# SAIC-MONTREAL/multimodal-dynamics

Measured on AMD Instinct MI355X. Metric: visuotactile samples/sec (train) + ELBO vs CPU ref, cnn-mvae 64x64 bs256 @1/2/4/8 GPU, higher is better.
Workload: dtype f32x3; 1 GPU; cnn-mvae visuotactile+pose 64x64, bs=256 per GPU, fp32 storage and results, GEMMs in the fp32x3 arithmetic (exact three-term bf16 split of the fp32 operands, six of nine products on the bf16 matrix cores, fp32 accumulate; error vs fp64 <= native fp32 MFMA), seq_modeling train step (7 subset ELBOs + backward + Adam), BASELINE configs[1]; global_batch=256, parallelism=dp1, bn=local, launch=hip_graph

## Files before the change

### include/mmdyn_hip.h

```cpp
#ifndef MMDYN_HIP_H
#define MMDYN_HIP_H

#include <stdint.h>

#ifdef __cplusplus
extern "C" {
#endif

#define MMDYN_OK 0
#define MMDYN_ERR_SHAPE (-1)
#define MMDYN_ERR_NULL (-2)
#define MMDYN_ERR_RANGE (-3)

#define MMDYN_ACT_NONE 0
#define MMDYN_ACT_SWISH 1
#define MMDYN_ACT_RELU 2

#define MMDYN_DENSE 0
#define MMDYN_CONV 1
#define MMDYN_TCONV_S2P1 2
#define MMDYN_IM2COL3 3

#define MMDYN_TCONV_S1P0 4

// ... 26 lines not shown
int mmdyn_igemm_stat_tiles(int mode, int G, int Bg, int Hi, int Wi, int Cin, int Ho, int Wo, int N);
int mmdyn_igemm_stat_tiles_bf16(int mode, int G, int Bg, int Hi, int Wi, int Cin, int Ho, int Wo, int N);
int mmdyn_igemm_stat_tiles_mx(int mode, int G, int Bg, int Hi, int Wi, int Cin, int Ho, int Wo, int N, int flags);
int mmdyn_igemm_slab_floats_mx(int mode, int G, int Bg, int Hi, int Wi, int Cin, int Ho, int Wo, int N, int flags);
int mmdyn_igemm_nt_grouped(const void* A, const void* Bp, const float* bias, void* C, void* C_act, const void* u, int G,
                           int rows, int K, int N, int act, int flags, void* stream);
int mmdyn_splitk_reduce(const float* ws, const float* bias, float* C, float* C_act, int splitk,
                        int rows, int N, int act, void* stream);

int mmdyn_wgrad_tn(const float* D, const float* Gt, float* partial, int mode, int Bt, int Hr, int Wr,
                   int Cd, int Hi, int Wi, int Cg, int stride, int offset, int chunks, void* stream);
int mmdyn_wgrad_tn_bf16(const float* D, const float* Gt, float* partial, int mode, int Bt, int Hr, int Wr,
                        int Cd, int Hi, int Wi, int Cg, int stride, int offset, int chunks, void* stream);
int mmdyn_wgrad_tn_f16(const float* D, const float* Gt, float* partial, int mode, int Bt, int Hr, int Wr,
                       int Cd, int Hi, int Wi, int Cg, int stride, int offset, int chunks, void* stream);
int mmdyn_wgrad_tn_grouped(const void* D, const void* Gt, float* partial, int G, int rows, int Cd, int Cg, int chunks,
                           int flags, void* stream);
int mmdyn_wgrad_out3_bn(const void* y, const float* mean, const float* rstd, const float* gamma, const float* beta,
                        const float* Gt, float* partial, int G, int Bg, int Hr, int chunks, int y_b16, void* stream);
int mmdyn_wgrad_chunks(int mode, int rows, int Cd, int Cg);
int mmdyn_wgrad_chunks_mx(int mode, int rows, int Cd, int Cg, int flags);
int mmdyn_wgrad_reduce(const float* partial, float* canon, int chunks, int taps, int Cd, int Cg,
                       int cg_canon, int perm, float beta, void* stream);

int mmdyn_pack_conv_weight(const float* Wc, float* P, int d0, int d1, int swap, void* stream);
int mmdyn_repack2d(const float* in, float* out, int rows_in, int cols_in, int rows_out, int cols_out,
                   int mode, void* stream);

int mmdyn_repack2d_ld(const float* in, float* out, int rows_in, int cols_in, int rows_out, int cols_out,
                      int ld_out, int mode, void* stream);
int mmdyn_pack_conv_weight_b16(const float* Wc, void* P, int d0, int d1, int swap, int half, void* stream);
int mmdyn_repack2d_ld_b16(const float* in, void* out, int rows_in, int cols_in, int rows_out, int cols_out,
                          int ld_out, int mode, int half, void* stream);
typedef struct {
  const float* src;
  float* dst;
  int kind, rows_in, cols_in, rows_out, cols_out, ld_out;
  int dst_bf16;
} mmdyn_pack_entry;
int mmdyn_pack_plan(const mmdyn_pack_entry* plan_dev, int n, void* stream);

int mmdyn_im2col_nchw3(const float* x, float* col, int Bt, int H, int W, void* stream);
int mmdyn_col2im_k4(const float* col, float* out, int Bt, int Hi, int Wi, int Ho, int Wo, int C,
                    int ldcol, int stride, int pad, int tap_major, void* stream);

int mmdyn_tconv_out3_fwd(const float* a, const float* w, float* out, int Bt, int Hi, int Wi, void* stream);
// ... 268 lines not shown
```

### multimodal-dynamics_amd/csrc/wgrad_geom.h

```cpp
#pragma once
#include "common.h"

struct WgradGeom {
  int d_b16, g_b16;
  int f16;
  int mode;
  int rows;
  int Hr, Wr, Cd;
  int Hi, Wi, Cg;
  int rs, ro;
  int ntaps, chunks, rows_per_chunk;
  int groups;
  int x3;
  int pre;
};

#ifdef MMDYN_LAB
int mmdyn_wgrad_ws_try(const float* D, const float* Gt, float* partial, const WgradGeom& g, hipStream_t st);
#else
static inline int mmdyn_wgrad_ws_try(const float*, const float*, float*, const WgradGeom&, hipStream_t) { return 1; }
#endif

int mmdyn_wgrad_p3_try(const void* D, const void* Gt, float* partial, const WgradGeom& g, int Bt, hipStream_t st);
int mmdyn_wgrad_p3_chunks(int rows, int Cd, int Cg);
```

### multimodal-dynamics_amd/csrc/wgrad_tn.hip

```cpp
#include <stdlib.h>
#include "common.h"
#include "wgrad_geom.h"

namespace {


constexpr int RK = 32;

typedef __bf16 bf16x4 __attribute__((ext_vector_type(4)));
typedef short s16x4 __attribute__((ext_vector_type(4)));
typedef _Float16 f16x4 __attribute__((ext_vector_type(4)));
__device__ __forceinline__ f16x4 pack4_f16(float a, float b, float c, float d) {
  f16x4 r;
  r[0] = (_Float16)a; r[1] = (_Float16)b; r[2] = (_Float16)c; r[3] = (_Float16)d;
  return r;
}
__device__ __forceinline__ s16x4 pack4_bf16(float a, float b, float c, float d) {
  bf16x4 r;
  r[0] = (__bf16)a; r[1] = (__bf16)b; r[2] = (__bf16)c; r[3] = (__bf16)d;
  return __builtin_bit_cast(s16x4, r);
}

template <int BX> struct x3_ld { static constexpr int v = (BX == 32) ? 32 : BX + 32; };
template <int MODE, int BD, int BG, int WD, int WG, int WK, bool BF16, int ST, bool X3 = false, int PRE = 0>
__global__ __launch_bounds__(256) void wgrad_tn_kernel(const float* __restrict__ D,
                                                       const float* __restrict__ Gt,
                                                       float* __restrict__ partial, const WgradGeom g) {
  static_assert(!X3 || (!BF16 && ST == 0 && WK == 1 && MODE != MMDYN_IM2COL3), "the three-term split is a variant of the fp32 kernel");
  static_assert(PRE == 0 || X3, "operands that arrive split belong to the three-term split arithmetic");
  constexpr bool PD = (PRE & 1) != 0, PG = (PRE & 2) != 0;
  constexpr int DT = WD / 32, GT = WG / 32;
  constexpr int WAVES_G = BG / WG;
  constexpr int WAVES_DG = (BD / WD) * WAVES_G;
  static_assert(WAVES_DG * WK == 4, "4 waves per block");
  constexpr int KPW = (RK / 2) / WK;
  constexpr int DV = BD / 4, GV = BG / 4;
  constexpr int D_LOADS = (RK * DV) / 256, G_LOADS = (RK * GV) / 256;
  static_assert(D_LOADS >= 1 && G_LOADS >= 1, "tile too small for 256 threads");

  extern __shared__ __attribute__((aligned(16))) char smem[];
  float* Ds = reinterpret_cast<float*>(smem);
  float* Gs = Ds + RK * BD;
  constexpr int LDD = x3_ld<BD>::v, LDG = x3_ld<BG>::v;
  bf16_t* Ds16 = reinterpret_cast<bf16_t*>(smem);
  bf16_t* Gs16 = Ds16 + 3 * RK * LDD;

  const int tid = threadIdx.x, lane = tid & 63, wave = tid >> 6;
  const int wk = wave / WAVES_DG, wdg = wave % WAVES_DG;
  const int wd = wdg / WAVES_G, wg = wdg % WAVES_G;
  const int tiles_g = g.Cg / BG;
  const int td = blockIdx.x / tiles_g, tg = blockIdx.x - td * tiles_g;
  const int cd0 = td * BD, cg0 = tg * BG;
  const int tap = blockIdx.y;
  const int ngrp = g.groups > 1 ? g.groups : 1;
  const int zb = gridDim.z / ngrp;
  const int grp = blockIdx.z / zb, chunk = blockIdx.z - grp * zb;
  const int dh = (MODE == MMDYN_CONV) ? (tap >> 2) : 0;
  const int dw = (MODE == MMDYN_CONV) ? (tap & 3) : 0;
  const int HWr = g.Hr * g.Wr;

  const int row_begin = grp * g.rows + chunk * g.rows_per_chunk;
  const int row_end = min((grp + 1) * g.rows, row_begin + g.rows_per_chunk);

  const float inv_hw = 1.0f / (float)HWr, inv_w = 1.0f / (float)g.Wr;
  auto fdiv = [](int n, int d, float inv, int& q, int& r) {
    q = (int)((float)n * inv);
    r = n - q * d;
    if (r < 0) { q -= 1; r += d; }
    if (r >= d) { q += 1; r -= d; }
  };
  f32x4 rd[D_LOADS], rg[G_LOADS];
  constexpr int DV8 = BD / 8, GV8 = BG / 8;
  constexpr int D_LOADS8 = (RK * DV8) / 256, G_LOADS8 = (RK * GV8) / 256;
  static_assert(PRE == 0 || (D_LOADS8 >= 1 && G_LOADS8 >= 1), "plane granules: tile too small for 256 threads");
  u32x4 pd[PD ? D_LOADS8 : 1][3], pg[PG ? G_LOADS8 : 1][3];
  unsigned okd = 0, okg = 0;
  auto gload = [&](int r0) {
    if constexpr (PD) {
#pragma unroll
      for (int i = 0; i < D_LOADS8; ++i) {
        const int idx = tid + 256 * i;
        const int r = idx / DV8, v = idx - r * DV8;
        const int row = r0 + r;
        const bool ok = row < row_end;
        const bf16_t* b = reinterpret_cast<const bf16_t*>(D) + (size_t)(ok ? row : 0) * 3 * g.Cd + cd0 + v * 8;
// ... 139 lines not shown
    }
#pragma unroll
    for (int i = 0; i < D_LOADS; ++i)
      reinterpret_cast<f32x4*>(Ds)[tid + 256 * i] = ((okd >> i) & 1u) ? rd[i] : zero;
#pragma unroll
    for (int i = 0; i < G_LOADS; ++i) {
      const unsigned m = okg >> (4 * i);
      f32x4 v;
      v[0] = (m & 1u) ? rg[i][0] : 0.f;
      v[1] = (m & 2u) ? rg[i][1] : 0.f;
      v[2] = (m & 4u) ? rg[i][2] : 0.f;
      v[3] = (m & 8u) ? rg[i][3] : 0.f;
      reinterpret_cast<f32x4*>(Gs)[tid + 256 * i] = v;
    }
  };

  f32x16 acc[DT][GT];
#pragma unroll
  for (int a = 0; a < DT; ++a)
#pragma unroll
    for (int b = 0; b < GT; ++b)
#pragma unroll
      for (int e = 0; e < 16; ++e) acc[a][b][e] = 0.f;

  const int h = lane >> 5, cl = lane & 31;
  if (row_begin < row_end) {
    gload(row_begin);
    lds_store();
    __syncthreads();
    for (int r0 = row_begin; r0 < row_end; r0 += RK) {
      gload(r0 + RK);
      __builtin_amdgcn_sched_barrier(0);
      if constexpr (X3) {
        const int gq = lane >> 4, tq = (lane >> 2) & 3, tp = lane & 3;
        const int trow = 8 * (gq >> 1) + tq, tcol = 16 * (gq & 1) + 4 * tp;
        typedef __attribute__((address_space(3))) s16x4* lds_s16x4_p;
        typedef __bf16 xb16x8 __attribute__((ext_vector_type(8)));
        auto frag = [&](const bf16_t* tile, int ld, int col0, int k0) {
          const s16x4 lo = __builtin_amdgcn_ds_read_tr16_b64_v4i16((lds_s16x4_p)(&tile[(k0 + trow) * ld + col0 + tcol]));
          const s16x4 hi = __builtin_amdgcn_ds_read_tr16_b64_v4i16((lds_s16x4_p)(&tile[(k0 + trow + 4) * ld + col0 + tcol]));
          typedef short s16x8 __attribute__((ext_vector_type(8)));
          const s16x8 v = {lo[0], lo[1], lo[2], lo[3], hi[0], hi[1], hi[2], hi[3]};
          return __builtin_bit_cast(xb16x8, v);
        };
#pragma unroll
        for (int kc = 0; kc < 2; ++kc) {
// ... 47 lines not shown
            pb[b] = pack4_bf16(p[0], p[BG], p[2 * BG], p[3 * BG]);
          }
#pragma unroll
          for (int a = 0; a < DT; ++a)
#pragma unroll
            for (int b = 0; b < GT; ++b)
              acc[a][b] = __builtin_amdgcn_mfma_f32_32x32x8bf16_1k(pa[a], pb[b], acc[a][b], 0, 0, 0);
          }
        }
      } else
#pragma unroll
      for (int kk = wk * KPW; kk < (wk + 1) * KPW; ++kk) {
        float af[DT], bf[GT];
#pragma unroll
        for (int a = 0; a < DT; ++a) af[a] = Ds[(2 * kk + h) * BD + wd * WD + a * 32 + cl];
#pragma unroll
        for (int b = 0; b < GT; ++b) bf[b] = Gs[(2 * kk + h) * BG + wg * WG + b * 32 + cl];
#pragma unroll
        for (int a = 0; a < DT; ++a)
#pragma unroll
          for (int b = 0; b < GT; ++b)
            acc[a][b] = __builtin_amdgcn_mfma_f32_32x32x2f32(af[a], bf[b], acc[a][b], 0, 0, 0);
      }
      __builtin_amdgcn_sched_barrier(0);
      __syncthreads();
      lds_store();
      __syncthreads();
    }
  }

  float* out = partial + ((size_t)(((chunk * WK + wk) * ngrp + grp) * g.ntaps + tap) * g.Cd) * g.Cg;
#pragma unroll
  for (int a = 0; a < DT; ++a)
#pragma unroll
    for (int e = 0; e < 16; ++e) {
      const int cd = cd0 + wd * WD + a * 32 + (e & 3) + 8 * (e >> 2) + 4 * h;
#pragma unroll
      for (int b = 0; b < GT; ++b) {
        const int cg = cg0 + wg * WG + b * 32 + cl;
        out[(size_t)cd * g.Cg + cg] = acc[a][b][e];
      }
    }
}

typedef __bf16 wb16x8 __attribute__((ext_vector_type(8)));
typedef _Float16 wf16x8 __attribute__((ext_vector_type(8)));
typedef float wacc16_t __attribute__((ext_vector_type(16)));
template <bool H16> __device__ __forceinline__ wacc16_t mfma16(wb16x8 a, wb16x8 b, wacc16_t c) {
  if constexpr (H16)
    return __builtin_amdgcn_mfma_f32_32x32x16_f16(__builtin_bit_cast(wf16x8, a), __builtin_bit_cast(wf16x8, b), c, 0, 0, 0);
  else
// ... 624 lines not shown
  for (int64_t tile = blockIdx.x; tile < ntiles; tile += gridDim.x) {
    const int64_t i = tile * 32 + il;
    float s0 = 0.f, s1 = 0.f, s2 = 0.f, s3 = 0.f;
    if (i < slab) {
      int c = cl;
      for (; c + 24 < chunks; c += 32) {
        s0 += partial[(size_t)c * slab + i];
        s1 += partial[(size_t)(c + 8) * slab + i];
        s2 += partial[(size_t)(c + 16) * slab + i];
        s3 += partial[(size_t)(c + 24) * slab + i];
      }
      for (; c < chunks; c += 8) s0 += partial[(size_t)c * slab + i];
    }
    red[cl][il] = (s0 + s1) + (s2 + s3);
    __syncthreads();
    if (cl == 0 && i < slab) {
      float s = 0.f;
#pragma unroll
      for (int k = 0; k < 8; ++k) s += red[k][il];
      int cg = (int)(i % Cg);
      int64_t t = i / Cg;
      int cd = (int)(t % Cd);
      int tap = (int)(t / Cd);
      if (cg < cg_canon) {
        int64_t o;
        if (perm == 0) {
          o = ((int64_t)cd * cg_canon + cg) * taps + tap;
        } else if (perm == 1) {
          int hw = cg / 256, ch = cg - hw * 256;
          o = (int64_t)cd * cg_canon + ch * 25 + hw;
        } else {
          int hw = cd / 256, ch = cd - hw * 256;
          o = (int64_t)(ch * 25 + hw) * cg_canon + cg;
        }
        canon[o] = (beta != 0.f) ? (beta * canon[o] + s) : s;
      }
    }
    __syncthreads();
  }
}

__global__ __launch_bounds__(256) void wgrad_reduce_vec_kernel(const float* __restrict__ partial,
                                                               float* __restrict__ canon, int chunks, int taps,
                                                               int Cd, int Cg, int cg_canon, int perm, float beta) {
  const int64_t slab = (int64_t)taps * Cd * Cg, nvec = slab >> 2;
  for (int64_t v = blockIdx.x * (int64_t)blockDim.x + threadIdx.x; v < nvec; v += (int64_t)gridDim.x * blockDim.x) {
    const int64_t i = v << 2;
    f32x4 s = {0.f, 0.f, 0.f, 0.f};
#pragma unroll 8
    for (int c = 0; c < chunks; ++c) s += *reinterpret_cast<const f32x4*>(partial + (size_t)c * slab + i);
    const int cg0 = (int)(i % Cg);
    const int64_t t = i / Cg;
    const int cd = (int)(t % Cd), tap = (int)(t / Cd);
#pragma unroll
    for (int k = 0; k < 4; ++k) {
      const int cg = cg0 + k;
      if (cg >= cg_canon) continue;
      int64_t o;
      if (perm == 0) {
        o = ((int64_t)cd * cg_canon + cg) * taps + tap;
      } else if (perm == 1) {
        int hw = cg / 256, ch = cg - hw * 256;
        o = (int64_t)cd * cg_canon + ch * 25 + hw;
      } else {
        int hw = cd / 256, ch = cd - hw * 256;
        o = (int64_t)(ch * 25 + hw) * cg_canon + cg;
      }
      canon[o] = (beta != 0.f) ? (beta * canon[o] + s[k]) : s[k];
    }
  }
}

template <int BD, int BG, int WD, int WG, int WK>
static int launch_b16(const float* D, const float* Gt, float* partial, WgradGeom g, hipStream_t st) {
  const int zblocks = g.chunks / WK;
  int rpc = ceil_div(g.rows, zblocks);
  g.rows_per_chunk = ceil_div(rpc, RK) * RK;
  dim3 grid((unsigned)((g.Cd / BD) * (g.Cg / BG) * g.ntaps) * (unsigned)((zblocks + 7) / 8 * 8));
#define WGRAD_B16(M, H)                                                                                    \
  hipLaunchKernelGGL((wgrad_b16_kernel<M, BD, BG, WD, WG, WK, H>), grid, dim3(256), 0, st,                 \
                     reinterpret_cast<const bf16_t*>(D), reinterpret_cast<const bf16_t*>(Gt), partial, g)
  if (g.mode == MMDYN_CONV) {
    if (g.f16) WGRAD_B16(MMDYN_CONV, true);
    else WGRAD_B16(MMDYN_CONV, false);
  } else {
    if (g.f16) WGRAD_B16(MMDYN_DENSE, true);
    else WGRAD_B16(MMDYN_DENSE, false);
  }
#undef WGRAD_B16
  MMDYN_LAUNCH_CHECK();
}
// ... 31 lines not shown
      MMDYN_LAUNCH_CHECK();
    }
  }
#define WGRAD_LAUNCH(M, BF, ST_)                                                                                      \
  hipLaunchKernelGGL((wgrad_tn_kernel<M, BD, BG, WD, WG, WK, BF, ST_>), grid, dim3(256), smem, st, D, Gt, partial, g)
#define WGRAD_MODE(M)                                                  \
  do {                                                                 \
    if (bf16 && g.f16 && g.d_b16 && g.g_b16) WGRAD_LAUNCH(M, true, 5); \
    else if (bf16 && g.f16 && g.d_b16) WGRAD_LAUNCH(M, true, 6);       \
    else if (bf16 && g.f16 && g.g_b16) WGRAD_LAUNCH(M, true, 7);       \
    else if (bf16 && g.d_b16 && g.g_b16) WGRAD_LAUNCH(M, true, 1);     \
    else if (bf16 && g.d_b16) WGRAD_LAUNCH(M, true, 2);                \
    else if (bf16 && g.g_b16) WGRAD_LAUNCH(M, true, 3);                \
    else if (bf16 && g.f16) WGRAD_LAUNCH(M, true, 4);                  \
    else if (bf16) WGRAD_LAUNCH(M, true, 0);                           \
    else WGRAD_LAUNCH(M, false, 0);                                    \
  } while (0)
  if (g.mode == MMDYN_CONV) WGRAD_MODE(MMDYN_CONV);
  else if (g.mode == MMDYN_DENSE) WGRAD_MODE(MMDYN_DENSE);
  else if constexpr (BG == 64) WGRAD_MODE(MMDYN_IM2COL3);
  else return MMDYN_ERR_SHAPE;
#undef WGRAD_MODE
#undef WGRAD_LAUNCH
  MMDYN_LAUNCH_CHECK();
}

}

static bool tile_128x64() {
  const char* e = lab_env("MMDYN_WGRAD_128x64");
  return !(e && e[0] == '0');
}

static bool p3_enabled() {
  const char* e = lab_env("MMDYN_WGRAD_P3");
  return !(e && e[0] == '0');
}

static bool p3_asked(bool x3, int pre, int mode) { return x3 && pre == 3 && mode == MMDYN_CONV && p3_enabled(); }

enum WgradFamily {
  WGRAD_TN,
  WGRAD_TN4,
  WGRAD_B16
};
struct WgradRoute {
// ... 157 lines not shown
    if (c > 0) return c;
  }
  return wgrad_chunks_impl(mode, rows, Cd, Cg, (flags & 6) == 6, x3);
}

extern "C" int mmdyn_wgrad_reduce(const float* partial, float* canon, int chunks, int taps, int Cd, int Cg,
                                  int cg_canon, int perm, float beta, void* stream) {
  if (!partial || !canon) return MMDYN_ERR_NULL;
  if (cg_canon > Cg || cg_canon <= 0) return MMDYN_ERR_SHAPE;
  if (perm == 1 && (Cg % 256 || Cg / 256 != 25)) return MMDYN_ERR_SHAPE;
  if (perm == 2 && (Cd % 256 || Cd / 256 != 25)) return MMDYN_ERR_SHAPE;
  int64_t slab = (int64_t)taps * Cd * Cg;
  if (chunks <= 64 && slab >= 65536) {
    hipLaunchKernelGGL(wgrad_reduce_vec_kernel, dim3(ew_grid(slab >> 2)), dim3(256), 0, (hipStream_t)stream, partial,
                       canon, chunks, taps, Cd, Cg, cg_canon, perm, beta);
    MMDYN_LAUNCH_CHECK();
  }
  int64_t ntiles = (slab + 31) / 32;
  int grid = (int)(ntiles < 8192 ? ntiles : 8192);
  hipLaunchKernelGGL(wgrad_reduce_kernel, dim3(grid), dim3(256), 0, (hipStream_t)stream, partial, canon, chunks,
                     taps, Cd, Cg, cg_canon, perm, beta);
  MMDYN_LAUNCH_CHECK();
}
```

### multimodal-dynamics_amd/mmdyn_hip/_lib.py

```python
import ctypes
import os

_HERE = os.path.dirname(os.path.abspath(__file__))
LIB_PATH = os.environ.get("MMDYN_HIP_LIB") or os.path.join(_HERE, "libmmdyn_hip.so")

_P, _I, _L, _F, _Q = ctypes.c_void_p, ctypes.c_int, ctypes.c_int64, ctypes.c_float, ctypes.c_uint64


class PassExperts(ctypes.Structure):
    _fields_ = [("mu", _P * 4), ("lv", _P * 4), ("dmu", _P * 4), ("dlv", _P * 4), ("ld", _I * 4), ("dz", _P * 3),
                ("zdst", _P * 3), ("zpl", _P * 3)]


class PackEntry(ctypes.Structure):
    _fields_ = [("src", _P), ("dst", _P), ("kind", _I), ("rows_in", _I), ("cols_in", _I), ("rows_out", _I),
                ("cols_out", _I), ("ld_out", _I), ("dst_bf16", _I)]


class FeedGroups(ctypes.Structure):
    _fields_ = [("recon", _P * 4), ("obs", _P * 4), ("out", _P * 4), ("row_len", _I * 4), ("logits", _I * 4), ("column", _I * 4)]


class GatherGroups(ctypes.Structure):
    _fields_ = [("src", _P * 4), ("out", _P * 4), ("row_len", _I * 4), ("logits", _I * 4)]
# ... 10 lines not shown
ABI_VERSION = 6

_SIGNATURES = {
    "mmdyn_abi_version": "",
    "mmdyn_igemm_nt": "ppppppp" + "iiiiiiiiiiiiii" + "p",
    "mmdyn_igemm_nt_dgrad_bn": "ppppppppp" + "iiiiiiiiiiii" + "ppp",
    "mmdyn_igemm_nt_dgrad_act": "pppp" + "i" + "iiiiiiiiiii" + "i" + "ppp",
    "mmdyn_igemm_slab_floats": "iiiiiiiii",
    "mmdyn_igemm_nt_bf16": "ppppppp" + "iiiiiiiiiiiiii" + "p",
    "mmdyn_igemm_nt_f16": "ppppppp" + "iiiiiiiiiiiiii" + "p",
    "mmdyn_igemm_stat_tiles": "iiiiiiiii",
    "mmdyn_igemm_stat_tiles_bf16": "iiiiiiiii",
    "mmdyn_igemm_stat_tiles_mx": "iiiiiiiiii",
    "mmdyn_igemm_slab_floats_mx": "iiiiiiiiii",
    "mmdyn_igemm_nt_grouped": "pppppp" + "iiiiii" + "p",
    "mmdyn_splitk_reduce": "pppp" + "iiii" + "p",
    "mmdyn_wgrad_tn": "ppp" + "iiiiiiiiiii" + "p",
    "mmdyn_wgrad_tn_bf16": "ppp" + "iiiiiiiiiii" + "p",
    "mmdyn_wgrad_tn_f16": "ppp" + "iiiiiiiiiii" + "p",
    "mmdyn_wgrad_tn_grouped": "ppp" + "iiiiii" + "p",
    "mmdyn_wgrad_chunks": "iiii",
    "mmdyn_wgrad_chunks_mx": "iiiii",
    "mmdyn_wgrad_reduce": "pp" + "iiiiii" + "f" + "p",
    "mmdyn_pack_conv_weight": "pp" + "iii" + "p",
    "mmdyn_repack2d": "pp" + "iiiii" + "p",
    "mmdyn_repack2d_ld": "pp" + "iiiiii" + "p",
    "mmdyn_pack_conv_weight_b16": "pp" + "iiii" + "p",
    "mmdyn_repack2d_ld_b16": "pp" + "iiiiiii" + "p",
    "mmdyn_pack_plan": "p" + "i" + "p",
    "mmdyn_im2col_nchw3": "pp" + "iii" + "p",
    "mmdyn_col2im_k4": "pp" + "iiiiiiiiii" + "p",
    "mmdyn_tconv_out3_fwd": "ppp" + "iii" + "p",
    "mmdyn_tconv_out3_bn_fwd": "ppppppp" + "iiiii" + "p",
    "mmdyn_tconv_out3_bn_bce": "ppppppp" + "i" + "pp" + "i" + "pppp" + "f" + "iiiii" + "p",
    "mmdyn_wgrad_out3_bn": "ppppppp" + "iiiii" + "p",
    "mmdyn_colstats": "pp" + "iii" + "p",
    "mmdyn_colstats_tiles": "i",
    "mmdyn_bn_finalize": "ppppppp" + "iiii" + "ff" + "i" + "pp",
    "mmdyn_bn_swish_fwd": "pppppp" + "iii" + "p",
    "mmdyn_bn_swish_bwd_reduce": "ppppppp" + "iii" + "p",
    "mmdyn_bn_bwd_finalize": "ppppp" + "iii" + "f" + "pp",
    "mmdyn_bn_eval_stats": "pppp" + "ii" + "f" + "p",
    "mmdyn_bn_reduce_partials": "ppp" + "iii" + "p",
    "mmdyn_bn_finalize_sums": "pppppp" + "iii" + "ff" + "i" + "p",
    "mmdyn_bn_bwd_finalize_sums": "pppp" + "ii" + "ff" + "p",
    "mmdyn_bn_swish_bwd_apply": "pppppppp" + "iiii" + "p",
# ... 125 lines not shown
```

### multimodal-dynamics_amd/mmdyn_hip/layers.py

```python
import weakref

import torch

from . import ops
from .ops import ACT_NONE, ACT_SWISH, ACT_RELU, DENSE, CONV, TCONV_S2P1, IM2COL3, TCONV_S1P0
from .models.shapes import BN_EPS, BN_MOMENTUM, FEAT


def _new(like, *shape, dtype=torch.float32):
    if isinstance(like, ops.Planes):
        like = like.t
    return torch.empty(shape, device=like.device, dtype=dtype)


ACT_DTYPE = torch.float32
W_DTYPE = torch.float32


def _act(like, *shape):
    return torch.empty(shape, device=like.device, dtype=ACT_DTYPE)


def _cdiv(a, b):
    return (a + b - 1) // b
# ... 33 lines not shown
    else:
        ops.B.igemm_nt(A, Bp, bias, C, Ca, None, None, DENSE, 1, rows, 1, 1, K, 1, 1, N, N, 1, 0, act, 1)
    return C, Ca


PLANES = True
PLANE_TWIN = {}


def _plane_twin(Wp):
    ent = PLANE_TWIN.get(Wp.data_ptr())
    if ent is None:
        return None
    if ent[0]() is not Wp:
        if ent[0]() is None:
            del PLANE_TWIN[Wp.data_ptr()]
        return None
    return ent[1]


PATCH_PLANES = True
CONV1_PLANES = True
OUT3_RECOMPUTE = True


def _conv3_plane_op(name, switch, S, *tensors):
    if not switch or S != 64 or ACT_DTYPE != torch.float32 or any(t.dtype != torch.float32 for t in tensors):
        return None
    return getattr(ops.B, name, None)


def planes_served(mode, G, Bg, Hi, Cin, Ho, N):
    served = getattr(ops.B, "igemm_planes_served", None) if PLANES else None
    if N == 32 and not PATCH_PLANES:
        return False
    return bool(served is not None and ACT_DTYPE == torch.float32 and served(mode, G, Bg, Hi, Hi, Cin, Ho, Ho, N))


def split_operands(x, Wp, mode, G, Bg, Hi, Cin, Ho, N):
    if isinstance(Wp, ops.Planes):
        return x, Wp
    xin = x.t if isinstance(x, ops.Planes) else x
    if xin.dtype not in (torch.float32, torch.bfloat16) or Wp.dtype != torch.float32 or not planes_served(mode, G, Bg, Hi, Cin, Ho, N):
        if isinstance(x, ops.Planes):
            raise ValueError("mmdyn_hip: a plane operand for a launch the plane-ring kernel does not serve")
        return x, Wp
# ... 221 lines not shown
            _bn_eval_param_grads(y, partial, T, dgamma, dbeta, G, N)
        dy, dyp = _apply_out(y, planes_out)
        ops.backend_op("bn_eval_swish_bwd")(du, None, mean, rstd, bn.gamma, bn.beta, dy, None, G, rows_per_group, N, True, planes=dyp)
        return dy if dyp is None else dyp
    sums = _bn_backward_sums(y, partial, T, dgamma, dbeta, G, N)
    dy, dyp = _apply_out(y, planes_out)
    if dyp is not None:
        ops.B.bn_swish_bwd_apply(du, y, mean, rstd, bn.gamma, bn.beta, sums, None, G, rows_per_group, N, True, planes=dyp)
        return dyp
    ops.B.bn_swish_bwd_apply(du, y, mean, rstd, bn.gamma, bn.beta, sums, dy, G, rows_per_group, N, True)
    return dy


def wgrad(D, Gt, canon, mode, Bt, Hr, Cd, Hi, Cg, stride=1, offset=0, cg_canon=None, perm=0, defer=None):
    if defer is not None:
        defer.append((D, Gt, canon, mode, Bt, Hr, Cd, Hi, Cg, stride, offset, cg_canon, perm))
        return
    rows = Bt * Hr * Hr
    taps = 16 if mode == CONV else 1
    if isinstance(D, ops.Planes) or isinstance(Gt, ops.Planes):
        chunks = ops.B.wgrad_chunks(mode, rows, Cd, Cg, planes=(isinstance(D, ops.Planes), isinstance(Gt, ops.Planes)))
    else:
        chunks = ops.B.wgrad_chunks(mode, rows, Cd, Cg)
    partial = _new(D, chunks, taps, Cd, Cg)
    ops.B.wgrad_tn(D, Gt, partial, mode, Bt, Hr, Hr, Cd, Hi, Hi, Cg, stride, offset, chunks)
    ops.B.wgrad_reduce(partial, canon, chunks, taps, Cd, Cg, Cg if cg_canon is None else cg_canon, perm, 0.0)


def run_deferred_wgrads(queue):
    while queue:
        item = queue.pop(0)
        if item and callable(item[0]):
            item[0](*item[1:])
        else:
            wgrad(*item)


def bn_stats_only(y, partial, T, bn, G, rows_per_group, C, repeat=1):
    if partial is None:
        return _eval_stats(y, bn, G, C)
    return _bn_forward_stats(y, partial, T, bn, G, rows_per_group, C, repeat)


def fuses_last_bn(S):
    return S in (64, 128, 256)

# ... 686 lines not shown
```

### multimodal-dynamics_amd/mmdyn_hip/ops.py

```python
import ctypes

import os

import torch

from . import _lib
from ._lib import PassExperts, FeedGroups, GatherGroups, EnsembleGroups, MAX_PASSES, MAX_EXPERTS, FEED_GROUPS, check

ACT_NONE, ACT_SWISH, ACT_RELU = 0, 1, 2
DENSE, CONV, TCONV_S2P1, IM2COL3, TCONV_S1P0 = 0, 1, 2, 3, 4
ROW_GROUPS_MAX = 8
PLAN_TOP_MAX = 8
REFIT_N_MAX = 4096


def _ptr(t, dtype=torch.float32):
    if t is None:
        return None
    if not t.is_cuda:
        raise RuntimeError("mmdyn_hip: the HIP path needs GPU tensors (got a CPU tensor); there is no CPU fallback")
    if t.dtype != dtype:
        raise TypeError(f"mmdyn_hip: expected {dtype}, got {t.dtype}")
    if not t.is_contiguous():
        raise ValueError("mmdyn_hip: tensor must be contiguous")
# ... 330 lines not shown
                else:
                    ptrs.append(_ptr(t))
            check(self.lib.mmdyn_wgrad_tn_mx(ptrs[0], ptrs[1], _ptr(partial), mode, Bt, Hr, Wr, Cd, Hi, Wi, Cg, stride, offset, chunks,
                                             flags, _stream()), "mmdyn_wgrad_tn_mx")
            return
        (pd, d16), (pg, g16) = _aptr(D), _aptr(Gt)
        if d16 or g16:
            check(self.lib.mmdyn_wgrad_tn_mx(pd, pg, _ptr(partial), mode, Bt, Hr, Wr, Cd, Hi, Wi, Cg, stride, offset, chunks,
                                             self._mx(d16, g16) | (2 if d16 else 0) | (4 if g16 else 0), _stream()),
                  "mmdyn_wgrad_tn_mx")
            return
        if self._x3():
            check(self.lib.mmdyn_wgrad_tn_mx(pd, pg, _ptr(partial), mode, Bt, Hr, Wr, Cd, Hi, Wi, Cg, stride, offset, chunks, 128,
                                             _stream()), "mmdyn_wgrad_tn_mx")
            return
        fn = {"fp32": self.lib.mmdyn_wgrad_tn, "fp16": self.lib.mmdyn_wgrad_tn_f16,
              "fp16s": self.lib.mmdyn_wgrad_tn_f16}.get(self.precision, self.lib.mmdyn_wgrad_tn_bf16)
        check(fn(pd, pg, _ptr(partial), mode, Bt, Hr, Wr, Cd, Hi, Wi, Cg, stride, offset, chunks,
                 _stream()), "mmdyn_wgrad_tn")

    def wgrad_reduce(self, partial, canon, chunks, taps, Cd, Cg, cg_canon, perm, beta):
        check(self.lib.mmdyn_wgrad_reduce(_ptr(partial), _ptr(canon), chunks, taps, Cd, Cg, cg_canon, perm,
                                          float(beta), _stream()), "mmdyn_wgrad_reduce")

    def pack_conv_weight(self, Wc, P, d0, d1, swap):
        pp, p16 = _aptr(P)
        if p16:
            check(self.lib.mmdyn_pack_conv_weight_b16(_ptr(Wc), pp, d0, d1, int(swap), _half(p16), _stream()),
                  "mmdyn_pack_conv_weight_b16")
            return
        check(self.lib.mmdyn_pack_conv_weight(_ptr(Wc), pp, d0, d1, int(swap), _stream()), "mmdyn_pack_conv_weight")

    def repack2d(self, src, dst, rows_in, cols_in, rows_out, cols_out, mode):
        if _is16(dst):
            return self.repack2d_ld(src, dst, rows_in, cols_in, rows_out, cols_out, cols_out, mode)
        check(self.lib.mmdyn_repack2d(_ptr(src), _ptr(dst), rows_in, cols_in, rows_out, cols_out, mode, _stream()),
              "mmdyn_repack2d")

    def repack2d_ld(self, src, dst, rows_in, cols_in, rows_out, cols_out, ld_out, mode):
        _, d16 = _aptr(dst)
        if d16:
            check(self.lib.mmdyn_repack2d_ld_b16(_ptr(src), dst.data_ptr(), rows_in, cols_in, rows_out, cols_out, ld_out, mode,
                                                 _half(d16), _stream()), "mmdyn_repack2d_ld_b16")
            return
        check(self.lib.mmdyn_repack2d_ld(_ptr(src), dst.data_ptr(), rows_in, cols_in, rows_out, cols_out, ld_out, mode,
                                         _stream()), "mmdyn_repack2d_ld")
# ... 966 lines not shown
```

### multimodal-dynamics_amd/mmdyn_hip/profiling.py

```python
import collections

import torch

from . import ops

PAD_CYCLES = 100000
HOST_ONLY = {"igemm_stat_tiles", "colstats_tiles", "wgrad_chunks", "igemm_planes_served"}


def _canon(name, a):
    if name == "igemm_nt_dgrad_bn":
        A, Bp, C, stats, y, mean, rstd, gamma, beta, mode, G, Bg, Hi, Wi, Cin, Ho, Wo, N, stride, offset = a
        name, a = "igemm_nt", (A, Bp, y, C, None, stats, None, mode, G, Bg, Hi, Wi, Cin, Ho, Wo, N, N, stride, offset, 0, 1)
    if name == "igemm_nt_dgrad_act":
        A, Bp, C, u, act, mode, G, Bg, Hi, Wi, Cin, Ho, Wo, N, stride, offset = a
        name, a = "igemm_nt", (A, Bp, u, C, None, None, None, mode, G, Bg, Hi, Wi, Cin, Ho, Wo, N, N, stride, offset, 0, 1)
    if name == "igemm_nt_grouped":
        A, Bp, bias, C, C_act, u, G, rows, K, N, act = a
        name, a = "igemm_nt", (A, Bp, bias if u is None else u, C, C_act, None, None, ops.DENSE, G, rows, 1, 1, K, 1, 1, N, N, 1, 0, act, 1)
    if name == "wgrad_tn_grouped":
        D, Gt, partial, G, rows, Cd, Cg, chunks = a
        name, a = "wgrad_tn", (D, Gt, partial, ops.DENSE, G * rows, 1, 1, Cd, 1, 1, Cg, 1, 0, chunks)
    if name == "wgrad_out3_bn":
        y, mean, rstd, gamma, beta, Gt, partial, G, Bg, Hr, chunks = a
        return "conv3_wgrad", (y, Gt, partial, ops.IM2COL3, G * Bg, Hr, Hr, 32, 2 * Hr, 2 * Hr, 64, 1, 0, chunks)
    if name == "tconv_out3_bn_fwd":
        return "tconv_out3_fwd", a
    if name == "conv3_fwd_planes":
        x, Wp, C, planes, G, Bg, H, act = a
        return "conv3_nt", (x, Wp, None, C, planes, None, None, ops.IM2COL3, G, Bg, H, H, 64, H // 2, H // 2, 32, 32, 1, 0, act, 1)
    if name == "conv3_dgrad_bn_stats":
        x, Wp, stats, y, mean, rstd, gamma, beta, G, Bg, H = a
        return "conv3_nt", (x, Wp, y, None, None, stats, None, ops.IM2COL3, G, Bg, H, H, 64, H // 2, H // 2, 32, 32, 1, 0, 0, 1)
    if name == "conv3_dgrad_bn_apply_planes":
        x, Wp, y, mean, rstd, gamma, beta, sums, planes, G, Bg, H = a
        return "conv3_nt", (x, Wp, y, planes, None, None, None, ops.IM2COL3, G, Bg, H, H, 64, H // 2, H // 2, 32, 32, 1, 0, 0, 1)
    if name == "igemm_nt" and a[7] == ops.IM2COL3 and a[10] in (64, 128, 256) and \
            tuple(a[10:17]) == (a[10], a[10], 64, a[10] // 2, a[10] // 2, 32, 32):
        return "conv3_nt", a
    if name == "igemm_nt" and a[7] == ops.TCONV_S2P1 and tuple(a[10:16]) in ((16, 16, 64, 32, 32, 32), (32, 32, 32, 64, 64, 32),
                                                                            (64, 64, 32, 128, 128, 32)) and \
            getattr(ops.B, "precision", "fp32") == "fp32" and all(not torch.is_tensor(t) or t.dtype == torch.float32 for t in a[:4]):
        return "tconv_patch", a
    if name == "wgrad_tn" and a[3] == ops.IM2COL3 and a[8] in (64, 128, 256) and \
            tuple(a[5:11]) == (a[8] // 2, a[8] // 2, 32, a[8], a[8], 64):
# ... 107 lines not shown
```

Baseline: 53740 samples/s.

## Fuse dense wgrad split-K reduction into a single canonical-output kernel

Adds a 'once' variant of the dense weight-gradient kernel. Each block walks all rows of its tile instead of one chunk, folds the accumulators at chunk boundaries to keep the same summation order, and writes straight into the canonical (permuted) weight-gradient layout. This removes the partial-buffer write, the separate reduce launch and their HBM traffic for perm==1 dense layers. In exchange there is much less grid parallelism (no chunk dimension), partly offset by an XCD-aware block ordering.

```diff
diff --git a/include/mmdyn_hip.h b/include/mmdyn_hip.h
--- a/include/mmdyn_hip.h
+++ b/include/mmdyn_hip.h
@@ -72,6 +72,9 @@
 int mmdyn_wgrad_chunks_mx(int mode, int rows, int Cd, int Cg, int flags);
 int mmdyn_wgrad_reduce(const float* partial, float* canon, int chunks, int taps, int Cd, int Cg,
                        int cg_canon, int perm, float beta, void* stream);
+int mmdyn_wgrad_tn_canon(const void* D, const void* Gt, float* canon, int G, int rows, int Cd, int Cg, int cg_canon, int perm,
+                         float beta, int chunks, int flags, void* stream);
+int mmdyn_wgrad_canon_served(int rows, int Cd, int Cg, int groups, int flags);
 
 int mmdyn_pack_conv_weight(const float* Wc, float* P, int d0, int d1, int swap, void* stream);
 int mmdyn_repack2d(const float* in, float* out, int rows_in, int cols_in, int rows_out, int cols_out,
diff --git a/multimodal-dynamics_amd/csrc/wgrad_geom.h b/multimodal-dynamics_amd/csrc/wgrad_geom.h
--- a/multimodal-dynamics_amd/csrc/wgrad_geom.h
+++ b/multimodal-dynamics_amd/csrc/wgrad_geom.h
@@ -13,6 +13,9 @@
   int groups;
   int x3;
   int pre;
+  int cg_canon, perm;
+  float beta;
+  int xcd_order;
 };
 
 #ifdef MMDYN_LAB
diff --git a/multimodal-dynamics_amd/csrc/wgrad_tn.hip b/multimodal-dynamics_amd/csrc/wgrad_tn.hip
--- a/multimodal-dynamics_amd/csrc/wgrad_tn.hip
+++ b/multimodal-dynamics_amd/csrc/wgrad_tn.hip
@@ -1,4 +1,5 @@
 #include <stdlib.h>
+#include <string.h>
 #include "common.h"
 #include "wgrad_geom.h"
 
@@ -6,6 +7,19 @@
 
 
 constexpr int RK = 32;
+
+__device__ __forceinline__ int64_t canon_index(int tap, int cd, int cg, int taps, int cg_canon, int perm) {
+  if (perm == 0) return ((int64_t)cd * cg_canon + cg) * taps + tap;
+  if (perm == 1) {
+    const int hw = cg / 256, ch = cg - hw * 256;
+    return (int64_t)cd * cg_canon + ch * 25 + hw;
+  }
+  const int hw = cd / 256, ch = cd - hw * 256;
+  return (int64_t)(ch * 25 + hw) * cg_canon + cg;
+}
+__device__ __forceinline__ void canon_store(float* __restrict__ canon, int64_t o, float s, float beta) {
+  canon[o] = (beta != 0.f) ? (beta * canon[o] + s) : s;
+}
 
 typedef __bf16 bf16x4 __attribute__((ext_vector_type(4)));
 typedef short s16x4 __attribute__((ext_vector_type(4)));
@@ -22,12 +36,13 @@
 }
 
 template <int BX> struct x3_ld { static constexpr int v = (BX == 32) ? 32 : BX + 32; };
-template <int MODE, int BD, int BG, int WD, int WG, int WK, bool BF16, int ST, bool X3 = false, int PRE = 0>
+template <int MODE, int BD, int BG, int WD, int WG, int WK, bool BF16, int ST, bool X3 = false, int PRE = 0, bool ONCE = false>
 __global__ __launch_bounds__(256) void wgrad_tn_kernel(const float* __restrict__ D,
                                                        const float* __restrict__ Gt,
                                                        float* __restrict__ partial, const WgradGeom g) {
   static_assert(!X3 || (!BF16 && ST == 0 && WK == 1 && MODE != MMDYN_IM2COL3), "the three-term split is a variant of the fp32 kernel");
   static_assert(PRE == 0 || X3, "operands that arrive split belong to the three-term split arithmetic");
+  static_assert(!ONCE || (MODE == MMDYN_DENSE && WK == 1 && PRE == 0 && (ST == 0 || ST == 4)), "the once form: dense, fp32 operands in HBM");
   constexpr bool PD = (PRE & 1) != 0, PG = (PRE & 2) != 0;
   constexpr int DT = WD / 32, GT = WG / 32;
   constexpr int WAVES_G = BG / WG;
@@ -49,18 +64,42 @@
   const int wk = wave / WAVES_DG, wdg = wave % WAVES_DG;
   const int wd = wdg / WAVES_G, wg = wdg % WAVES_G;
   const int tiles_g = g.Cg / BG;
-  const int td = blockIdx.x / tiles_g, tg = blockIdx.x - td * tiles_g;
+  const int ngrp = g.groups > 1 ? g.groups : 1;
+  int td, tg, tap, grp, chunk;
+  if constexpr (ONCE) {
+    const int tiles = (g.Cd / BD) * tiles_g, n = tiles * ngrp;
+    int v = blockIdx.x;
+    if (g.xcd_order) {
+      const int per = (n + 7) >> 3;
+      v = (v & 7) * per + (v >> 3);
+      if (v >= n) return;
+    }
+    grp = v / tiles;
+    const int t = v - grp * tiles;
+    if (g.perm == 1) {
+      constexpr int TPH = 256 / BG;
+      const int hw = t % 25, rest = t / 25;
+      td = rest / TPH;
+      tg = hw * TPH + (rest - td * TPH);
+    } else {
+      td = t / tiles_g;
+      tg = t - td * tiles_g;
+    }
+    tap = 0;
+    chunk = 0;
+  } else {
+    td = blockIdx.x / tiles_g, tg = blockIdx.x - td * tiles_g;
+    tap = blockIdx.y;
+    const int zb = gridDim.z / ngrp;
+    grp = blockIdx.z / zb, chunk = blockIdx.z - grp * zb;
+  }
   const int cd0 = td * BD, cg0 = tg * BG;
-  const int tap = blockIdx.y;
-  const int ngrp = g.groups > 1 ? g.groups : 1;
-  const int zb = gridDim.z / ngrp;
-  const int grp = blockIdx.z / zb, chunk = blockIdx.z - grp * zb;
   const int dh = (MODE == MMDYN_CONV) ? (tap >> 2) : 0;
   const int dw = (MODE == MMDYN_CONV) ? (tap & 3) : 0;
   const int HWr = g.Hr * g.Wr;
 
   const int row_begin = grp * g.rows + chunk * g.rows_per_chunk;
-  const int row_end = min((grp + 1) * g.rows, row_begin + g.rows_per_chunk);
+  const int row_end = ONCE ? (grp + 1) * g.rows : min((grp + 1) * g.rows, row_begin + g.rows_per_chunk);
 
   const float inv_hw = 1.0f / (float)HWr, inv_w = 1.0f / (float)g.Wr;
   auto fdiv = [](int n, int d, float inv, int& q, int& r) {
@@ -246,6 +285,16 @@
     for (int b = 0; b < GT; ++b)
 #pragma unroll
       for (int e = 0; e < 16; ++e) acc[a][b][e] = 0.f;
+  f32x16 tot[ONCE ? DT : 1][ONCE ? GT : 1];
+  if constexpr (ONCE) {
+#pragma unroll
+    for (int a = 0; a < DT; ++a)
+#pragma unroll
+      for (int b = 0; b < GT; ++b)
+#pragma unroll
+        for (int e = 0; e < 16; ++e) tot[a][b][e] = 0.f;
+  }
+  int fold_at = row_begin + g.rows_per_chunk;
 
   const int h = lane >> 5, cl = lane & 31;
   if (row_begin < row_end) {
@@ -339,11 +388,42 @@
           for (int b = 0; b < GT; ++b)
             acc[a][b] = __builtin_amdgcn_mfma_f32_32x32x2f32(af[a], bf[b], acc[a][b], 0, 0, 0);
       }
+      if constexpr (ONCE) {
+        if (r0 + RK == fold_at) {
+          fold_at += g.rows_per_chunk;
+#pragma unroll
+          for (int a = 0; a < DT; ++a)
+#pragma unroll
+            for (int b = 0; b < GT; ++b)
+#pragma unroll
+              for (int e = 0; e < 16; ++e) {
+                tot[a][b][e] += acc[a][b][e];
+                acc[a][b][e] = 0.f;
+              }
+        }
+      }
       __builtin_amdgcn_sched_barrier(0);
       __syncthreads();
       lds_store();
       __syncthreads();
     }
+  }
+
+  if constexpr (ONCE) {
+    const int cgc = g.cg_canon, perm = g.perm;
+    const float beta = g.beta;
+#pragma unroll
+    for (int a = 0; a < DT; ++a)
+#pragma unroll
+      for (int e = 0; e < 16; ++e) {
+        const int cd = grp * g.Cd + cd0 + wd * WD + a * 32 + (e & 3) + 8 * (e >> 2) + 4 * h;
+#pragma unroll
+        for (int b = 0; b < GT; ++b) {
+          const int cg = cg0 + wg * WG + b * 32 + cl;
+          if (cg < cgc) canon_store(partial, canon_index(0, cd, cg, 1, cgc, perm), tot[a][b][e] + acc[a][b][e], beta);
+        }
+      }
+    return;
   }
 
   float* out = partial + ((size_t)(((chunk * WK + wk) * ngrp + grp) * g.ntaps + tap) * g.Cd) * g.Cg;
@@ -1014,19 +1094,7 @@
       int64_t t = i / Cg;
       int cd = (int)(t % Cd);
       int tap = (int)(t / Cd);
-      if (cg < cg_canon) {
-        int64_t o;
-        if (perm == 0) {
-          o = ((int64_t)cd * cg_canon + cg) * taps + tap;
-        } else if (perm == 1) {
-          int hw = cg / 256, ch = cg - hw * 256;
-          o = (int64_t)cd * cg_canon + ch * 25 + hw;
-        } else {
-          int hw = cd / 256, ch = cd - hw * 256;
-          o = (int64_t)(ch * 25 + hw) * cg_canon + cg;
-        }
-        canon[o] = (beta != 0.f) ? (beta * canon[o] + s) : s;
-      }
+      if (cg < cg_canon) canon_store(canon, canon_index(tap, cd, cg, taps, cg_canon, perm), s, beta);
     }
     __syncthreads();
   }
@@ -1048,17 +1116,7 @@
     for (int k = 0; k < 4; ++k) {
       const int cg = cg0 + k;
       if (cg >= cg_canon) continue;
-      int64_t o;
-      if (perm == 0) {
-        o = ((int64_t)cd * cg_canon + cg) * taps + tap;
-      } else if (perm == 1) {
-        int hw = cg / 256, ch = cg - hw * 256;
-        o = (int64_t)cd * cg_canon + ch * 25 + hw;
-      } else {
-        int hw = cd / 256, ch = cd - hw * 256;
-        o = (int64_t)(ch * 25 + hw) * cg_canon + cg;
-      }
-      canon[o] = (beta != 0.f) ? (beta * canon[o] + s[k]) : s[k];
+      canon_store(canon, canon_index(tap, cd, cg, taps, cg_canon, perm), s[k], beta);
     }
   }
 }
@@ -1136,6 +1194,28 @@
   else return MMDYN_ERR_SHAPE;
 #undef WGRAD_MODE
 #undef WGRAD_LAUNCH
+  MMDYN_LAUNCH_CHECK();
+}
+
+template <int BD, int BG, int WD, int WG>
+static int launch_once(const float* D, const float* Gt, float* canon, WgradGeom g, hipStream_t st, bool bf16) {
+  const int rpc = ceil_div(g.rows, g.chunks);
+  g.rows_per_chunk = ceil_div(rpc, RK) * RK;
+  const int n = (g.Cd / BD) * (g.Cg / BG) * (g.groups > 1 ? g.groups : 1);
+  dim3 grid(g.xcd_order ? (n + 7) / 8 * 8 : n);
+  size_t smem = (size_t)RK * (BD + BG) * sizeof(float);
+#define WGRAD_ONCE(BF, ST_, X3_) \
+  hipLaunchKernelGGL((wgrad_tn_kernel<MMDYN_DENSE, BD, BG, WD, WG, 1, BF, ST_, X3_, 0, true>), grid, dim3(256), smem, st, D, Gt, canon, g)
+  if (g.x3 && !bf16) {
+    smem = (size_t)3 * RK * (x3_ld<BD>::v + x3_ld<BG>::v) * 2;
+    static LdsOptIn opt_in;
+    if (smem > 65536)
+      if (int e = opt_in.ensure((const void*)wgrad_tn_kernel<MMDYN_DENSE, BD, BG, WD, WG, 1, false, 0, true, 0, true>, (int)smem)) return e;
+    WGRAD_ONCE(false, 0, true);
+  } else if (bf16 && g.f16) WGRAD_ONCE(true, 4, false);
+  else if (bf16) WGRAD_ONCE(true, 0, false);
+  else WGRAD_ONCE(false, 0, false);
+#undef WGRAD_ONCE
   MMDYN_LAUNCH_CHECK();
 }
 
@@ -1339,3 +1419,64 @@
                      taps, Cd, Cg, cg_canon, perm, beta);
   MMDYN_LAUNCH_CHECK();
 }
+
+struct OnceTile {
+  int bd, bg;
+};
+static OnceTile once_tile(int Cd, int Cg) {
+  int want = 1;
+  if (const char* e = lab_env("MMDYN_WGRAD_ONCE_TILE")) want = !strcmp(e, "128x128") ? 3 : !strcmp(e, "128x64") ? 2 : 1;
+  const bool d128 = Cd % 128 == 0, g128 = Cg % 128 == 0;
+  if (want == 3 && d128 && g128) return {128, 128};
+  if (want >= 2 && d128) return {128, 64};
+  return {64, 64};
+}
+
+extern "C" int mmdyn_wgrad_canon_served(int rows, int Cd, int Cg, int groups, int flags) {
+  if (flags & ~(1 | 32 | 128)) return 0;
+  if ((flags & 128) && (flags & (1 | 32))) return 0;
+  if (rows <= 0 || groups < 1 || Cd <= 0 || Cg <= 0 || Cd % 32 || Cg % 32) return 0;
+  const WgradRoute r = wgrad_route(MMDYN_DENSE, Cd, Cg, false);
+  if (r.family != WGRAD_TN || r.wk != 1) return 0;
+  const int chunks = mmdyn_wgrad_chunks_mx(MMDYN_DENSE, rows, Cd, Cg, flags);
+  if (chunks < 4 || chunks > 64 || (int64_t)groups * Cd * Cg < 65536) return 0;
+  if ((int64_t)groups * rows * Cd >= (1LL << 31) || (int64_t)groups * rows * Cg >= (1LL << 31) || (int64_t)groups * Cd * Cg >= (1LL << 31)) return 0;
+  return 1;
+}
+
+extern "C" int mmdyn_wgrad_tn_canon(const void* D, const void* Gt, float* canon, int G, int rows, int Cd, int Cg, int cg_canon,
+                                    int perm, float beta, int chunks, int flags, void* stream) {
+  if (!D || !Gt || !canon) return MMDYN_ERR_NULL;
+  if (G < 1 || rows <= 0 || cg_canon > Cg || cg_canon <= 0 || perm < 0 || perm > 2) return MMDYN_ERR_SHAPE;
+  if (perm == 1 && (Cg % 256 || Cg / 256 != 25 || cg_canon != Cg)) return MMDYN_ERR_SHAPE;
+  if (perm == 2 && (Cd % 256 || Cd / 256 != 25)) return MMDYN_ERR_SHAPE;
+  if (perm != 0 && G > 1) return MMDYN_ERR_SHAPE;
+  if (chunks < 4 || chunks % 4 || chunks > 64) return MMDYN_ERR_SHAPE;
+  if (!mmdyn_wgrad_canon_served(rows, Cd, Cg, G, flags)) return MMDYN_ERR_SHAPE;
+  const bool bf16 = (flags & (1 | 32)) != 0;
+  bool x3 = (flags & 128) != 0;
+  if (const char* e = lab_env("MMDYN_X3_WGRAD")) x3 = e[0] == '1';
+  WgradGeom g{};
+  g.x3 = x3 && !bf16;
+  g.f16 = (flags & 32) != 0;
+  g.mode = MMDYN_DENSE;
+  g.groups = G;
+  g.rows = rows;
+  g.Hr = g.Wr = g.Hi = g.Wi = 1;
+  g.Cd = Cd;
+  g.Cg = Cg;
+  g.rs = 1;
+  g.ntaps = 1;
+  g.chunks = chunks;
+  g.cg_canon = cg_canon;
+  g.perm = perm;
+  g.beta = beta;
+  g.xcd_order = 1;
+  if (const char* e = lab_env("MMDYN_WGRAD_ONCE_XCD")) g.xcd_order = e[0] != '0';
+  hipStream_t st = (hipStream_t)stream;
+  const float *d = (const float*)D, *gt = (const float*)Gt;
+  const OnceTile t = once_tile(Cd, Cg);
+  if (t.bd == 128 && t.bg == 128) return launch_once<128, 128, 64, 64>(d, gt, canon, g, st, bf16);
+  if (t.bd == 128) return launch_once<128, 64, 64, 32>(d, gt, canon, g, st, bf16);
+  return launch_once<64, 64, 32, 32>(d, gt, canon, g, st, bf16);
+}
diff --git a/multimodal-dynamics_amd/mmdyn_hip/_lib.py b/multimodal-dynamics_amd/mmdyn_hip/_lib.py
--- a/multimodal-dynamics_amd/mmdyn_hip/_lib.py
+++ b/multimodal-dynamics_amd/mmdyn_hip/_lib.py
@@ -56,6 +56,8 @@
     "mmdyn_wgrad_chunks": "iiii",
     "mmdyn_wgrad_chunks_mx": "iiiii",
     "mmdyn_wgrad_reduce": "pp" + "iiiiii" + "f" + "p",
+    "mmdyn_wgrad_tn_canon": "ppp" + "iiiiii" + "f" + "ii" + "p",
+    "mmdyn_wgrad_canon_served": "iiiii",
     "mmdyn_pack_conv_weight": "pp" + "iii" + "p",
     "mmdyn_repack2d": "pp" + "iiiii" + "p",
     "mmdyn_repack2d_ld": "pp" + "iiiiii" + "p",
diff --git a/multimodal-dynamics_amd/mmdyn_hip/layers.py b/multimodal-dynamics_amd/mmdyn_hip/layers.py
--- a/multimodal-dynamics_amd/mmdyn_hip/layers.py
+++ b/multimodal-dynamics_amd/mmdyn_hip/layers.py
@@ -79,6 +79,8 @@
 PATCH_PLANES = True
 CONV1_PLANES = True
 OUT3_RECOMPUTE = True
+WGRAD_ONCE = True
+WGRAD_ONCE_PERMS = (1,)
 
 
 def _conv3_plane_op(name, switch, S, *tensors):
@@ -346,6 +348,11 @@
         chunks = ops.B.wgrad_chunks(mode, rows, Cd, Cg, planes=(isinstance(D, ops.Planes), isinstance(Gt, ops.Planes)))
     else:
         chunks = ops.B.wgrad_chunks(mode, rows, Cd, Cg)
+    if WGRAD_ONCE and mode == DENSE and perm in WGRAD_ONCE_PERMS:
+        once, served = getattr(ops.B, "wgrad_tn_canon", None), getattr(ops.B, "wgrad_canon_served", None)
+        if once is not None and served is not None and served(rows, Cd, Cg, 1, D, Gt):
+            once(D, Gt, canon, 1, rows, Cd, Cg, Cg if cg_canon is None else cg_canon, perm, 0.0, chunks)
+            return
     partial = _new(D, chunks, taps, Cd, Cg)
     ops.B.wgrad_tn(D, Gt, partial, mode, Bt, Hr, Hr, Cd, Hi, Hi, Cg, stride, offset, chunks)
     ops.B.wgrad_reduce(partial, canon, chunks, taps, Cd, Cg, Cg if cg_canon is None else cg_canon, perm, 0.0)
diff --git a/multimodal-dynamics_amd/mmdyn_hip/ops.py b/multimodal-dynamics_amd/mmdyn_hip/ops.py
--- a/multimodal-dynamics_amd/mmdyn_hip/ops.py
+++ b/multimodal-dynamics_amd/mmdyn_hip/ops.py
@@ -376,6 +376,21 @@
     def wgrad_reduce(self, partial, canon, chunks, taps, Cd, Cg, cg_canon, perm, beta):
         check(self.lib.mmdyn_wgrad_reduce(_ptr(partial), _ptr(canon), chunks, taps, Cd, Cg, cg_canon, perm,
                                           float(beta), _stream()), "mmdyn_wgrad_reduce")
+
+    def _wgrad_canon_flags(self):
+        return {"fp32": self._x3(), "fp16": 33, "fp16s": 33}.get(self.precision, 1)
+
+    def wgrad_canon_served(self, rows, Cd, Cg, groups=1, D=None, Gt=None):
+        if self.precision in ("bf16s", "fp16s"):
+            return False
+        for t in (D, Gt):
+            if isinstance(t, Planes) or (t is not None and t.dtype != torch.float32):
+                return False
+        return self.lib.mmdyn_wgrad_canon_served(rows, Cd, Cg, groups, self._wgrad_canon_flags()) == 1
+
+    def wgrad_tn_canon(self, D, Gt, canon, G, rows, Cd, Cg, cg_canon, perm, beta, chunks):
+        check(self.lib.mmdyn_wgrad_tn_canon(_ptr(D), _ptr(Gt), _ptr(canon), G, rows, Cd, Cg, cg_canon, perm, float(beta), chunks,
+                                            self._wgrad_canon_flags(), _stream()), "mmdyn_wgrad_tn_canon")
 
     def pack_conv_weight(self, Wc, P, d0, d1, swap):
         pp, p16 = _aptr(P)
diff --git a/multimodal-dynamics_amd/mmdyn_hip/profiling.py b/multimodal-dynamics_amd/mmdyn_hip/profiling.py
--- a/multimodal-dynamics_amd/mmdyn_hip/profiling.py
+++ b/multimodal-dynamics_amd/mmdyn_hip/profiling.py
@@ -5,7 +5,7 @@
 from . import ops
 
 PAD_CYCLES = 100000
-HOST_ONLY = {"igemm_stat_tiles", "colstats_tiles", "wgrad_chunks", "igemm_planes_served"}
+HOST_ONLY = {"igemm_stat_tiles", "colstats_tiles", "wgrad_chunks", "igemm_planes_served", "wgrad_canon_served"}
 
 
 def _canon(name, a):
@@ -21,6 +21,9 @@
     if name == "wgrad_tn_grouped":
         D, Gt, partial, G, rows, Cd, Cg, chunks = a
         name, a = "wgrad_tn", (D, Gt, partial, ops.DENSE, G * rows, 1, 1, Cd, 1, 1, Cg, 1, 0, chunks)
+    if name == "wgrad_tn_canon":
+        D, Gt, canon, G, rows, Cd, Cg, cg_canon, perm, beta, chunks = a
+        name, a = "wgrad_tn", (D, Gt, canon, ops.DENSE, G * rows, 1, 1, Cd, 1, 1, Cg, 1, 0, chunks)
     if name == "wgrad_out3_bn":
         y, mean, rstd, gamma, beta, Gt, partial, G, Bg, Hr, chunks = a
         return "conv3_wgrad", (y, Gt, partial, ops.IM2COL3, G * Bg, Hr, Hr, 32, 2 * Hr, 2 * Hr, 64, 1, 0, chunks)
```

Measured after the change: 54750 samples/s (median of 6 runs). 1.9% higher.
